# GStreamer/gstreamer

Measured on AMD Instinct MI355X. Metric: 4K frames/s (videoconvertscale NV12->BGRA) per GPU; % HBM roofline, higher is better.
Workload: dtype u8; 1 GPU; C2: 3840x2160 NV12 (bt709 limited, chroma-site mpeg2) -> BGRA, fused unpack + chroma upsample + matrix + pack, 32 frames/step, pools 33 in / 32 out resident in HBM, 1 stream per GPU, 32 frame(s) per kernel launch; plan=fused_convert_pair[NV12->BGRA,h2cs,v2,matrix=ayuv_argb], frames_per_launch=32, parallelism=stream-per-gpu x1

## Files before the change

### gstreamer_amd/csrc/video_scale_col.h

```cpp
#pragma once
#include "video_hscale420.h"

#define GSTAMD_COL_MAX_WAVES 8
#define GSTAMD_COL_MAX_FRAMES 16
#define GSTAMD_COL_FLAG_BYTES 64

namespace gstamd {

struct ColFrames {
  const uint8_t *y[GSTAMD_COL_MAX_FRAMES];
  const uint8_t *c0[GSTAMD_COL_MAX_FRAMES];
  const uint8_t *c1[GSTAMD_COL_MAX_FRAMES];
  uint8_t *dst[GSTAMD_COL_MAX_FRAMES];
};

#ifdef __HIPCC__
typedef __amdgpu_buffer_rsrc_t colplane_t;
#else
struct colplane_t { const uint8_t *p; uint32_t bytes; };
#endif
struct ColSrc {
  colplane_t y, c0, c1;
  colplane_t out;
};
// ... 478 lines not shown
       : "=&v" (w), "=&v" (t01), "=&v" (t23) : "s" (six), "v" (a0), "v" (a1), "v" (a2), "v" (a3));
  return w ^ 0x80808080u;
#else
  const int a[4] = {a0, a1, a2, a3};
  uint32_t w = 0;
  for (int k = 0; k < 4; k++) {
    const int v = ((int) (int16_t) (uint16_t) a[k]) >> 6;
    w |= (uint32_t) (v < 0 ? 0 : (v > 255 ? 255 : v)) << (8 * k);
  }
  return w ^ 0x80808080u;
#endif
}

GSTAMD_HD uint32_t col_fin_px (int ay, int au, int av)
{
#ifdef __HIPCC__
  uint32_t t01 = 0xffu, t23, w;
  const int six = 6;
  asm ("s_nop 2\n\t"
       "v_ashrrev_i16_sdwa %2, %3, %5 dst_sel:WORD_0 dst_unused:UNUSED_PAD src0_sel:DWORD src1_sel:WORD_0\n\t"
       "v_ashrrev_i16_sdwa %1, %3, %4 dst_sel:WORD_1 dst_unused:UNUSED_PRESERVE src0_sel:DWORD src1_sel:WORD_0\n\t"
       "v_ashrrev_i16_sdwa %2, %3, %6 dst_sel:WORD_1 dst_unused:UNUSED_PRESERVE src0_sel:DWORD src1_sel:WORD_0\n\t"
       "v_sat_pk_u8_i16 %0, %1\n\t"
       "v_sat_pk_u8_i16_sdwa %0, %2 dst_sel:WORD_1 dst_unused:UNUSED_PRESERVE src0_sel:DWORD\n\t"
       "s_nop 0"
       : "=&v" (w), "+v" (t01), "=&v" (t23) : "s" (six), "v" (ay), "v" (au), "v" (av));
  return w;
#else
  return 0xffu | (h420r_finish (ay) << 8) | (h420r_finish (au) << 16) | (h420r_finish (av) << 24);
#endif
}

template <int OPL, int NW, int WSTEP, int A8>
GSTAMD_HD void col_hfilter (const ColLane<OPL, NW> &L, const uint8_t *stage, uint32_t gw[3][OPL])
{
  typedef ColGeom<OPL> G;
  constexpr int SH = WSTEP >= 0 ? WSTEP : 0;
  constexpr int NWIN = WSTEP >= 0 ? 1 : OPL;
  constexpr int NWORDS = NW + SH;
  int acc[4][3][OPL];
  uint32_t w[2][3][NWIN][NWORDS];
  auto fetch = [&](int k, uint32_t (*d)[NWIN][NWORDS]) {
#pragma unroll
    for (int c = 0; c < 3; c++)
#pragma unroll
      for (int i = 0; i < NWIN; i++) {
#if defined(GSTAMD_COL_ABL) && GSTAMD_COL_ABL == 2
        for (int q = 0; q < NWORDS; q++)
          d[c][i][q] = (uint32_t) L.lb[k][i] * 3u + q + c;
#else
        col_lds_words<NWORDS, A8> (stage + L.lb[k][i] + c * G::PP, d[c][i]);
#endif
      }
  };
  fetch (0, w[0]);
#pragma unroll
  for (int k = 0; k < 4; k++) {
    if (k < 3)
      fetch (k + 1, w[(k + 1) & 1]);
#pragma unroll
    for (int c = 0; c < 3; c++)
#pragma unroll
      for (int i = 0; i < OPL; i++) {
        const uint32_t *ww = w[k & 1][c][WSTEP >= 0 ? 0 : i] + (WSTEP >= 0 && i ? SH : 0);
        int a = L.hinit[i];
#pragma unroll
        for (int q = 0; q < NW; q++) {
#if defined(GSTAMD_COL_ABL) && GSTAMD_COL_ABL == 5
          a ^= (int) ww[q];
#else
          a = col_dot4 (ww[q], L.tw[i][q], a);
#endif
        }
        acc[k][c][i] = a;
      }
  }
#pragma unroll
  for (int c = 0; c < 3; c++)
#pragma unroll
    for (int i = 0; i < OPL; i++)
      gw[c][i] = col_fin4 (acc[0][c][i], acc[1][c][i], acc[2][c][i], acc[3][c][i]);
}

template <int OPL, int NW, class NB>
GSTAMD_HD void col_hfilter_regs (const ColLane<OPL, NW> &L, NB &nb, uint32_t gw[3][OPL])
{
  static_assert (OPL == 2 && NW <= 4, "register windows: two outputs per lane, windows of up to five words");
  constexpr int NWORDS = NW + 1;
  int acc[4][3][OPL];
#pragma unroll
  for (int k = 0; k < 4; k++)
#pragma unroll
    for (int c = 0; c < 3; c++) {
      uint32_t w[5];
      w[0] = L.win[k][c][0], w[1] = L.win[k][c][1];
      w[2] = nb (w[0], k, c, 0, 1);
      w[3] = NWORDS > 3 ? nb (w[1], k, c, 1, 1) : 0u;
      w[4] = NWORDS > 4 ? nb (w[2], k, c, 0, 2) : 0u;
#pragma unroll
      for (int i = 0; i < OPL; i++) {
        int a = L.hinit[i];
#pragma unroll
        for (int q = 0; q < NW; q++)
          a = col_dot4 (w[q + i], L.tw[i][q], a);
        acc[k][c][i] = a;
      }
    }
#pragma unroll
  for (int c = 0; c < 3; c++)
#pragma unroll
    for (int i = 0; i < OPL; i++)
      gw[c][i] = col_fin4 (acc[0][c][i], acc[1][c][i], acc[2][c][i], acc[3][c][i]);
}

template <int OPL>
GSTAMD_HD void col_slot_store (uint32_t *slot, int lane, const uint32_t gw[3][OPL])
{
#pragma unroll
  for (int c = 0; c < 3; c++) {
    uint32_t *d = slot + (c * 64 + lane) * OPL;
    if constexpr (OPL == 2)
      *(uint2 *) d = gstamd_make_uint2 (gw[c][0], gw[c][1]);
    else
      *d = gw[c][0];
  }
}

template <int OPL>
GSTAMD_HD void col_slot_load (const uint32_t *slot, int lane, uint32_t gw[3][OPL])
{
#pragma unroll
  for (int c = 0; c < 3; c++) {
    const uint32_t *d = slot + (c * 64 + lane) * OPL;
    if constexpr (OPL == 2) {
      const uint2 v = *(const uint2 *) d;
      gw[c][0] = v.x, gw[c][1] = v.y;
    } else {
#ifdef __HIPCC__
      gw[c][0] = *(const __attribute__ ((address_space (3))) uint32_t *) d;
#else
      gw[c][0] = *d;
#endif
    }
  }
}

template <int OPL, int NGV>
GSTAMD_HD void col_ring_put (ColRingRegs<OPL, NGV> &rg, const uint32_t gw[3][OPL])
{
#pragma unroll
  for (int k = 0; k + 1 < NGV; k++)
#pragma unroll
    for (int c = 0; c < 3; c++)
#pragma unroll
      for (int i = 0; i < OPL; i++)
        rg.w[k][c][i] = rg.w[k + 1][c][i];
#pragma unroll
  for (int c = 0; c < 3; c++)
#pragma unroll
    for (int i = 0; i < OPL; i++)
      rg.w[NGV - 1][c][i] = gw[c][i];
}

template <int OPL, int NGV, int POST>
GSTAMD_HD void col_vrow (const ColRingRegs<OPL, NGV> &rg, const uint32_t *e, const ColParams &p, const ColSrc &s, const Dst &dst, const PostFast &pf, int x, int j)
{
  int acc[3][OPL];
#pragma unroll
  for (int c = 0; c < 3; c++)
#pragma unroll
    for (int i = 0; i < OPL; i++)
      acc[c][i] = (int) e[2];
#pragma unroll
  for (int k = 0; k < NGV; k++)
#pragma unroll
    for (int c = 0; c < 3; c++)
#pragma unroll
      for (int i = 0; i < OPL; i++)
        acc[c][i] = col_dot4s (rg.w[k][c][i], e[3 + k], acc[c][i]);
  uint32_t px[OPL];
#pragma unroll
  for (int i = 0; i < OPL; i++) {
    const uint32_t q = col_fin_px (acc[0][i], acc[1][i], acc[2][i]);
    if constexpr (POST) {
      const uint32_t z = q ^ 0x80808080u;
      px[i] = fast_pixel (pf.fp, z, 0x0c01010cu, z, 0x0c02020cu, 0x0c03030cu);
    } else {
      px[i] = dst.final ? pack_px (dst.pack_pos, apply_color (dst.post, q)) : q;
    }
  }
  col_store32 (s.out, (uint32_t) (4 * x), col_row_off (j, p.dstride), px, OPL);
}

struct ColWavePlan {
  int r0, r1;
  int ga, ge, gl, gp;
};

GSTAMD_HD bool col_wave_plan (const ColParams &p, int chunk, int wave, ColWavePlan *w)
{
  const int ra = chunk * p.rows_per_wg, rb = ra + p.rows_per_wg < p.out_h ? ra + p.rows_per_wg : p.out_h;
  w->r0 = ra + wave * p.rows_per_wave;
  if (w->r0 >= rb)
    return false;
  const int mine = wave == p.nwaves - 1 ? p.rows_last : p.rows_per_wave;
  w->r1 = w->r0 + mine < rb ? w->r0 + mine : rb;
  uint32_t e[8];
  col_entry8 (p.vrow, w->r0, e);
  w->ga = (int) e[0];
  col_entry8 (p.vrow, w->r1 - 1, e);
  w->gl = (int) e[1];
  if (w->r1 == rb || p.pubn == 0) {
    w->ge = w->gl + 1;
  } else {
    col_entry8 (p.vrow, w->r1, e);
    w->ge = (int) e[0];
    if (w->ge > w->gl + 1)
      w->ge = w->gl + 1;
  }
  if (w->r0 == ra || p.pubn == 0) {
    w->gp = w->ga - 1;
  } else {
    col_entry8 (p.vrow, w->r0 - 1, e);
    w->gp = (int) e[1];
  }
  return true;
}

template <int OPL, int NW, int NGV, int CH, int SEMI, int WSTEP, int A8, int POST, class X>
GSTAMD_HD void col_wave (X &x, const ColParams &p, const ColSrc &s, const int32_t *tile, const ColWavePlan &wp, uint8_t *wave_lds, uint8_t *below_lds,
    uint32_t *flags, int wave, const Dst &dst, const PostFast &pf)
{
  constexpr int RW = OPL == 2 && WSTEP == 1 && A8 == 2;
  typedef ColGeom<OPL, RW> G;
  typedef ColLane<OPL, NW> Lane;
  typedef ColRaw<OPL> Raw;
  typedef ColRingRegs<OPL, NGV> Ring;
  uint8_t *stage = wave_lds, *craw = wave_lds + G::STAGEB;
  uint32_t *pub = (uint32_t *) (wave_lds + G::STAGEB + GSTAMD_COL_CRAW_BYTES (OPL));
  const uint32_t *pub_below = (const uint32_t *) (below_lds + G::STAGEB + GSTAMD_COL_CRAW_BYTES (OPL));
  const bool aligned = ((tile[3] - tile[2]) % 16) == 0 && tile[3] > 0 && tile[3] + G::SPAN <= p.width;
  x.each ([&](int lane, Lane &L, Raw &ra, Ring &) {
    col_setup<OPL, NW, CH, SEMI, RW> (p, tile, lane, L);
    col_request_chroma<OPL, NW, SEMI> (p, s, L, 2 * wp.ga - 2, ra);
    if (aligned)
      col_stage_loads<OPL, NW, SEMI, 1, RW> (L, ra, stage, craw, false);
    else
      col_stage_loads<OPL, NW, SEMI, 0, RW> (L, ra, stage, craw, false);
    col_request<OPL, NW, SEMI> (p, s, L, wp.ga, ra);
  });
  x.sync ();
  x.each ([&](int, Lane &L, Raw &, Ring &) {
    if (aligned)
      col_first_row<OPL, NW, CH, SEMI, 1> (L, craw);
    else
      col_first_row<OPL, NW, CH, SEMI, 0> (L, craw);
  });
  x.sync ();
  int r = wp.r0;
  uint32_t e[8];
  col_entry8 (p.vrow, r, e);
#ifdef GSTAMD_COL_TRACE
  unsigned long long tacc[8] = {0, 0, 0, 0, 0, 0, 0, 0}, tprev = x.now ();
#define COL_STAMP(k) do { const unsigned long long t_ = x.now (); tacc[k] += t_ - tprev; tprev = t_; } while (0)
#else
#define COL_STAMP(k) do { } while (0)
#endif
  auto rows = [&](int g) {
    while (r < wp.r1 && (int) e[1] == g) {
#if !(defined(GSTAMD_COL_ABL) && GSTAMD_COL_ABL == 3)
      x.each ([&](int, Lane &L, Raw &, Ring &rg) { col_vrow<OPL, NGV, POST> (rg, e, p, s, dst, pf, L.xo, r); });
#endif
      r++;
      if (r < wp.r1)
        col_entry8 (p.vrow, r, e);
    }
  };
  int g = wp.ga;
  COL_STAMP (0);
  while (g < wp.ge) {
    const int gn = g + 1 < wp.ge ? g + 1 : wp.ge - 1;
#ifdef GSTAMD_COL_TRACE
    x.wait_loads ();
    COL_STAMP (1);
#endif
    if (aligned)
      x.each ([&](int, Lane &L, Raw &ra, Ring &) {
        col_stage_loads<OPL, NW, SEMI, 1, RW> (L, ra, stage, craw, true);
        col_request<OPL, NW, SEMI> (p, s, L, gn, ra);
      });
    else
      x.each ([&](int, Lane &L, Raw &ra, Ring &) {
        col_stage_loads<OPL, NW, SEMI, 0, RW> (L, ra, stage, craw, true);
        col_request<OPL, NW, SEMI> (p, s, L, gn, ra);
      });
    x.sync ();
    if (aligned)
      x.each ([&](int, Lane &L, Raw &, Ring &) { col_stage_chroma<OPL, NW, CH, SEMI, 1, RW> (L, craw, stage); });
    else
      x.each ([&](int, Lane &L, Raw &, Ring &) { col_stage_chroma<OPL, NW, CH, SEMI, 0, RW> (L, craw, stage); });
    x.sync ();
    COL_STAMP (2);
    if constexpr (RW) {
      x.each ([&](int, Lane &L, Raw &, Ring &) {
#pragma unroll
        for (int k = 0; k < 4; k++)
          col_lds_words<2, 1> (stage + L.st + k * G::LINEB, L.win[k][0]);
      });
      x.each_nb ([&](int lane, Lane &L, Raw &, Ring &rg, auto &nb) {
        uint32_t gw[3][OPL];
        col_hfilter_regs<OPL, NW> (L, nb, gw);
        col_ring_put<OPL, NGV> (rg, gw);
        if (g <= wp.gp)
          col_slot_store<OPL> (pub + (size_t) (g - wp.ga) * G::SLOTW, lane, gw);
      });
    } else {
      x.each ([&](int lane, Lane &L, Raw &, Ring &rg) {
        uint32_t gw[3][OPL];
        col_hfilter<OPL, NW, WSTEP, A8> (L, stage, gw);
        col_ring_put<OPL, NGV> (rg, gw);
        if (g <= wp.gp)
          col_slot_store<OPL> (pub + (size_t) (g - wp.ga) * G::SLOTW, lane, gw);
      });
    }
    x.sync ();
    if (g == wp.gp)
      x.publish (flags, wave);
    COL_STAMP (3);
    rows (g);
    COL_STAMP (4);
    g++;
  }
  if (wp.gp >= wp.ga)
    x.publish (flags, wave);
  if (wp.gl >= wp.ge) {
    x.wait_flag (flags, wave + 1);
    for (; g <= wp.gl; g++) {
      x.each ([&](int lane, Lane &, Raw &, Ring &rg) {
        uint32_t gw[3][OPL];
        col_slot_load<OPL> (pub_below + (size_t) (g - wp.ge) * G::SLOTW, lane, gw);
        col_ring_put<OPL, NGV> (rg, gw);
      });
      rows (g);
    }
  }
  COL_STAMP (5);
#ifdef GSTAMD_COL_TRACE
  x.trace_out (p.trace, tacc, wp.ge - wp.ga);
#endif
#undef COL_STAMP
}

}
```

### gstreamer_amd/csrc/video_fast.h

```cpp
#pragma once
#include "video_device.h"

namespace gstamd {

struct FastParams {
  int width, height;
  int p8[5];
  uint32_t pack_sel;
  int u_first;
  int pc[5];
  int crow_lo, crow_hi;
  int pack_pos[4];
  int px_bytes;
  const uint8_t *lut;
  int lut_keep;
  MatrixParams m8;
  int ayuv;
  int store_policy;
};

#ifdef __HIPCC__
extern __shared__ uint32_t fast_lut_lds[];
#else
static uint32_t fast_lut_lds[64];
// ... 205 lines not shown
#ifdef __HIPCC__
  uint32_t r;
  asm ("v_sat_pk_u8_i16 %0, %1" : "=v" (r) : "v" (v));
  return r;
#else
  const int a = (int16_t) (v & 0xffff), b = (int16_t) (v >> 16);
  return (uint32_t) (a < 0 ? 0 : a > 255 ? 255 : a) | ((uint32_t) (b < 0 ? 0 : b > 255 ? 255 : b) << 8);
#endif
}

GSTAMD_HD int add_hiwords (int pa, int pb)
{
#ifdef __HIPCC__
  int r;
  asm ("v_add_u32_sdwa %0, sext(%1), sext(%2) dst_sel:DWORD dst_unused:UNUSED_PAD src0_sel:WORD_1 src1_sel:WORD_1" : "=v" (r) : "v" (pa), "v" (pb));
  return r;
#else
  return (pa >> 16) + (pb >> 16);
#endif
}

template <int W>
GSTAMD_HD void add_hiwords_into (uint32_t &dst, int pa, int pb)
{
#ifdef __HIPCC__
  if (W == 0)
    asm ("v_add_u32_sdwa %0, sext(%1), sext(%2) dst_sel:WORD_0 dst_unused:UNUSED_PRESERVE src0_sel:WORD_1 src1_sel:WORD_1" : "+v" (dst) : "v" (pa), "v" (pb));
  else
    asm ("v_add_u32_sdwa %0, sext(%1), sext(%2) dst_sel:WORD_1 dst_unused:UNUSED_PRESERVE src0_sel:WORD_1 src1_sel:WORD_1" : "+v" (dst) : "v" (pa), "v" (pb));
#else
  const uint32_t r = (uint32_t) ((pa >> 16) + (pb >> 16)) & 0xffffu;
  dst = W == 0 ? (dst & 0xffff0000u) | r : (dst & 0x0000ffffu) | (r << 16);
#endif
}

GSTAMD_HD void sat_pk_u8_hi (uint32_t &dst, uint32_t v)
{
#ifdef __HIPCC__
  asm ("v_sat_pk_u8_i16_sdwa %0, %1 dst_sel:WORD_1 dst_unused:UNUSED_PRESERVE src0_sel:DWORD" : "+v" (dst) : "v" (v));
#else
  dst = (dst & 0xffffu) | (sat_pk_u8 (v) << 16);
#endif
}

GSTAMD_HD uint32_t pk_mad (uint32_t a, uint32_t k_splat, uint32_t c)
{
#ifdef __HIPCC__
  uint32_t r;
  asm ("v_pk_mad_u16 %0, %1, %2, %3" : "=v" (r) : "v" (a), "s" (k_splat), "v" (c));
  return r;
#else
  const uint32_t lo = ((a & 0xffffu) * (k_splat & 0xffffu) + (c & 0xffffu)) & 0xffffu;
  const uint32_t hi = ((a >> 16) * (k_splat >> 16) + (c >> 16)) & 0xffffu;
  return lo | (hi << 16);
#endif
}

GSTAMD_HD void blend_rows_hi (uint32_t a, uint32_t b, uint32_t &x0, uint32_t &x1)
{
  x0 = pk_mad (a, 0x00c000c0u, pk_mad (b, 0x00400040u, 0x80808080u));
  x1 = pk_mad (b, 0x00c000c0u, pk_mad (a, 0x00400040u, 0x80808080u));
}

#define GSTAMD_LAYOUT(pr, pg, pb) ((pr) | ((pg) << 2) | ((pb) << 4))
#define GSTAMD_LAYOUT_AYUV GSTAMD_LAYOUT (0, 0, 4)
#define GSTAMD_AYUV_X80(ys, c) ((bperm ((c), (ys), 0x0604000cu) ^ 0x80808000u) | 0xffu)
#define GSTAMD_AYUV_OUT(fp, px) ((fp).ayuv == 2 ? apply_matrix ((fp).m8, (px)) : (px))

template <int L>
GSTAMD_HD void layout_init (uint32_t (&q)[4][2])
{
  constexpr int PA = (L & GSTAMD_LAYOUT_AYUV) ? 0 : 6 - (L & 3) - ((L >> 2) & 3) - ((L >> 4) & 3);
#pragma unroll
  for (int j = 0; j < 4; j++) {
    q[j][0] = q[j][1] = 0;
    q[j][PA >> 1] = 255u << (16 * (PA & 1));
#ifdef __HIPCC__
    asm volatile ("" : "+v" (q[j][0]), "+v" (q[j][1]));
#endif
  }
}

template <int L, int ABL>
GSTAMD_HD void fast_emit4_l (const FastParams &fp, uint8_t *__restrict__ d, bool store, uint32_t yw, const uint32_t *xh, uint32_t (&q)[4][2])
{
  constexpr int PR = L & 3, PG = (L >> 2) & 3, PB = (L >> 4) & 3;
  uint32_t o[4];
  if (ABL == 1) {
#pragma unroll
    for (int j = 0; j < 4; j++)
      o[j] = yw ^ xh[j];
  } else {
    const uint32_t yx = yw ^ 0x80808080u;
    const uint32_t ys01 = bperm (yx, yx, 0x01010000u), ys23 = bperm (yx, yx, 0x03030202u);
    const uint32_t csel = fp.u_first ? 0x03030101u : 0x01010303u;
    uint32_t cs[4];
    int wy[4], prv[4], pbu[4], pgu[4], pgv[4], g0[4];
#pragma unroll
    for (int j = 0; j < 4; j++)
      cs[j] = bperm (xh[j], xh[j], csel);
    wy[0] = mul_word<0> (ys01, fp.pc[0]) + 0x00800000;
    wy[1] = mul_word<1> (ys01, fp.pc[0]) + 0x00800000;
    wy[2] = mul_word<0> (ys23, fp.pc[0]) + 0x00800000;
    wy[3] = mul_word<1> (ys23, fp.pc[0]) + 0x00800000;
#pragma unroll
    for (int j = 0; j < 4; j++)
      pgu[j] = mul_word<0> (cs[j], fp.pc[3]);
#pragma unroll
    for (int j = 0; j < 4; j++)
      prv[j] = mul_word<1> (cs[j], fp.pc[1]);
#pragma unroll
    for (int j = 0; j < 4; j++)
      g0[j] = add_hiwords (wy[j], pgu[j]);
#pragma unroll
    for (int j = 0; j < 4; j++)
      pgv[j] = mul_word<1> (cs[j], fp.pc[4]);
#pragma unroll
    for (int j = 0; j < 4; j++)
      add_hiwords_into<PR & 1> (q[j][PR >> 1], wy[j], prv[j]);
#pragma unroll
    for (int j = 0; j < 4; j++)
      pbu[j] = mul_word<0> (cs[j], fp.pc[2]);
#pragma unroll
    for (int j = 0; j < 4; j++)
      add_hiword_into<PG & 1> (q[j][PG >> 1], g0[j], pgv[j]);
#pragma unroll
    for (int j = 0; j < 4; j++)
      add_hiwords_into<PB & 1> (q[j][PB >> 1], wy[j], pbu[j]);
#pragma unroll
    for (int j = 0; j < 4; j++)
      o[j] = sat_pk_u8 (q[j][0]);
#pragma unroll
    for (int j = 0; j < 4; j++)
      sat_pk_u8_hi (o[j], q[j][1]);
  }
  if (ABL == GSTAMD_FAST_LUT) {
#pragma unroll
    for (int j = 0; j < 4; j++)
      o[j] = fast_lut3_px (o[j], fp.lut_keep);
  }
  if (store) {
    if (fp.px_bytes == 3)
      store12_stream (d, o[0], o[1], o[2], o[3]);
    else
      store16_policy (d, o[0], o[1], o[2], o[3], fp.store_policy);
  }
}

template <int CH>
GSTAMD_HD void chroma_filter4 (uint32_t raw, uint32_t nxt, uint32_t prv_hi, uint32_t *out)
{
  const uint32_t s1 = bperm (raw, raw, 0x0c010c00u), s2 = bperm (raw, raw, 0x0c030c02u);
  if (CH == CHROMA_H_NONE) {
    out[0] = out[1] = s1;
    out[2] = out[3] = s2;
    return;
  }
  const uint32_t s3 = bperm (nxt, nxt, 0x0c010c00u);
  if (CH == CHROMA_H_H2_CS) {
    out[0] = s1;
    out[1] = pk_shr<1> (s1 + s2 + 0x00010001u);
    out[2] = s2;
    out[3] = pk_shr<1> (s2 + s3 + 0x00010001u);
  } else {
    const uint32_t s0 = bperm (prv_hi, prv_hi, 0x0c030c02u);
    out[0] = pk_shr<2> (s0 + 3u * s1 + 0x00020002u);
    out[1] = pk_shr<2> (3u * s1 + s2 + 0x00020002u);
    out[2] = pk_shr<2> (s1 + 3u * s2 + 0x00020002u);
    out[3] = pk_shr<2> (3u * s2 + s3 + 0x00020002u);
  }
}

struct ChromaRaw4 {
  uint32_t raw, nxt, prv_hi;
};

struct __attribute__ ((aligned (4))) u32x2u { uint32_t a, b; };

GSTAMD_HD uint32_t load_stream32 (const uint8_t *__restrict__ p)
{
#ifdef __HIPCC__
  return __builtin_nontemporal_load ((const uint32_t *) p);
#else
  return *(const uint32_t *) p;
#endif
}

template <int CH>
GSTAMD_HD void chroma_load4 (const uint8_t *__restrict__ row, int cw, int x0, ChromaRaw4 &r)
{
  const int k0 = x0 >> 1;
  const uint8_t *p = row + 2 * (size_t) k0;
  r.nxt = r.prv_hi = 0;
  if (CH != CHROMA_H_NONE && k0 + 2 < cw) {
    const u32x2u m = *(const u32x2u *) p;
    r.raw = m.a;
    r.nxt = m.b;
  } else {
    r.raw = *(const uint32_t *) p;
    if (CH != CHROMA_H_NONE)
      r.nxt = *(const uint16_t *) (row + 2 * (size_t) (cw - 1));
  }
  if (CH == CHROMA_H_H2)
    r.prv_hi = (uint32_t) * (const uint16_t *) (row + 2 * (size_t) (k0 > 0 ? k0 - 1 : 0)) << 16;
}

template <int CH, int L, int ABL>
GSTAMD_HD void fast_strip (const FastParams &fp, const Planes &pl, uint8_t *__restrict__ dst, int dstride, int x0, int p_begin,
    int p_end)
{
  const int w = fp.width, h = fp.height, cw = (w + 1) >> 1;
  const uint8_t *yb = pl.p[0] + x0, *cbase = pl.p[1];
  const int ys = pl.stride[0], cs = pl.stride[1];
  uint8_t *db = dst + (size_t) fp.px_bytes * (size_t) x0;
  uint32_t q[4][2];
  layout_init<L> (q);

  uint32_t cprev[4], ccur[4], c0[4], c1[4];
  ChromaRaw4 craw;
  uint32_t y0, y1;
  {
    ChromaRaw4 r0;
    chroma_load4<CH> (cbase + (ptrdiff_t) (p_begin - 1 > fp.crow_lo ? p_begin - 1 : fp.crow_lo) * cs, cw, x0, r0);
    chroma_filter4<CH> (r0.raw, r0.nxt, r0.prv_hi, cprev);
  }
  {
    const int p = p_begin, l0 = 2 * p - 1, l1 = 2 * p;
    chroma_load4<CH> (cbase + (ptrdiff_t) (p < fp.crow_hi ? p : fp.crow_hi) * cs, cw, x0, craw);
    y0 = load_stream32 (yb + (size_t) (l0 >= 0 ? l0 : 0) * ys);
    y1 = load_stream32 (yb + (size_t) (l1 < h ? l1 : h - 1) * ys);
  }
  for (int p = p_begin; p < p_end; p++) {
    const int l0 = 2 * p - 1, l1 = 2 * p;
    const bool have0 = l0 >= 0, have1 = l1 < h;
    const uint32_t cy0 = y0, cy1 = y1;
    const ChromaRaw4 cr_now = craw;
    if (p + 1 < p_end) {
      const int pn = p + 1, n0 = 2 * pn - 1, n1 = 2 * pn;
      chroma_load4<CH> (cbase + (ptrdiff_t) (pn < fp.crow_hi ? pn : fp.crow_hi) * cs, cw, x0, craw);
      y0 = load_stream32 (yb + (size_t) n0 * ys);
      y1 = load_stream32 (yb + (size_t) (n1 < h ? n1 : h - 1) * ys);
    }
    chroma_filter4<CH> (cr_now.raw, cr_now.nxt, cr_now.prv_hi, ccur);
#pragma unroll
    for (int j = 0; j < 4; j++)
      blend_rows_hi (cprev[j], ccur[j], c0[j], c1[j]);
    fast_emit4_l<L, ABL> (fp, db + (size_t) (have0 ? l0 : l1) * dstride, have0, cy0, c0, q);
    fast_emit4_l<L, ABL> (fp, db + (size_t) (have1 ? l1 : l0) * dstride, have1, cy1, c1, q);
#pragma unroll
    for (int i = 0; i < 4; i++)
      cprev[i] = ccur[i];
  }
}

#define GSTAMD_WIDE_PX 1024
struct WideLds {
  uint32_t y[2][256];
  uint32_t c[2][4 + 256 + 4];
};

#ifdef __HIPCC__
typedef unsigned int gstamd_u32x4 __attribute__ ((ext_vector_type (4)));
#endif

template <bool STREAM>
GSTAMD_HD void wide_load16 (const uint8_t *__restrict__ p, int nd, bool vec, uint32_t *out)
{
  if (nd >= 4 && vec) {
#ifdef __HIPCC__
    const gstamd_u32x4 v = STREAM ? __builtin_nontemporal_load ((const gstamd_u32x4 *) p) : *(const gstamd_u32x4 *) p;
    out[0] = v.x;
    out[1] = v.y;
    out[2] = v.z;
    out[3] = v.w;
#else
    const uint4 v = *(const uint4 *) p;
    out[0] = v.x;
    out[1] = v.y;
    out[2] = v.z;
    out[3] = v.w;
#endif
  } else {
#pragma unroll
    for (int j = 0; j < 4; j++)
      out[j] = j < nd ? *(const uint32_t *) (p + 4 * j) : 0u;
  }
}

GSTAMD_HD void wide_put16 (uint32_t *l, const uint32_t *v)
{
  *(uint4 *) l = gstamd_make_uint4 (v[0], v[1], v[2], v[3]);
}

struct WideRegs {
  uint32_t y0[4], y1[4], c[4];
  uint32_t cn, cp;
};

template <int CH>
GSTAMD_HD void wide_fetch_chroma (const FastParams &fp, const Planes &pl, int xw, int crow, int lane, bool vec, WideRegs &r)
{
  const int w = fp.width, xl = xw + 16 * lane;
  if (xl >= w)
    return;
  const int nd = (w - xl) >> 2;
  const uint8_t *row = pl.p[1] + (ptrdiff_t) crow * pl.stride[1];
  wide_load16<false> (row + xl, nd, vec, r.c);
  if (CH != CHROMA_H_NONE && (lane == 63 || nd <= 4)) {
    const int xn = xl + 4 * (nd < 4 ? nd : 4);
    r.cn = xn < w ? *(const uint32_t *) (row + xn) : (uint32_t) * (const uint16_t *) (row + w - 2);
  }
  if (CH == CHROMA_H_H2 && lane == 0)
    r.cp = xw > 0 ? *(const uint32_t *) (row + xw - 4) : 0u;
}

template <int CH>
GSTAMD_HD void wide_commit_chroma (const FastParams &fp, int xw, int lane, const WideRegs &r, uint32_t *crow_lds)
{
  const int w = fp.width, xl = xw + 16 * lane;
  if (xl >= w)
    return;
  const int nd = (w - xl) >> 2;
  wide_put16 (&crow_lds[4 + 4 * lane], r.c);
  if (CH != CHROMA_H_NONE && (lane == 63 || nd <= 4))
    crow_lds[4 + 4 * lane + (nd < 4 ? nd : 4)] = r.cn;
  if (CH == CHROMA_H_H2 && lane == 0)
    crow_lds[3] = xw > 0 ? r.cp : r.c[0] << 16;
}

template <int CH>
GSTAMD_HD void wide_fetch (const FastParams &fp, const Planes &pl, int xw, int p, int lane, bool vec, WideRegs &r)
{
  const int w = fp.width, h = fp.height;
  const int xl = xw + 16 * lane;
  if (xl >= w)
    return;
  const int nd = (w - xl) >> 2;
// ... 60 lines not shown
```

### gstreamer_amd/csrc/video_kernels.hip

```cpp
#include <hip/hip_runtime.h>
#include <algorithm>
#include <cstdio>
#include <cstdlib>
#include <stdint.h>
#include <stdio.h>
#include <stdlib.h>
#include <string.h>

#include "planner.h"
#include "tuning.h"
#include "video_kernels.h"
#include "video_device.h"
#include "video_fast.h"
#include "video_scale_fast.h"
#include "video_hscale420.h"
#include "video_pack.h"
#include "video_bilinear_fast.h"
#include "video_encode_fast.h"
#include "video_planes.h"
#include "video_deep.h"
#include "video_dither.h"
#include "video_dither_ed.h"
#include "video_relayout.h"
#include "video_swizzle34.h"
// ... 1259 lines not shown
  if (vec_ok) {
    vec_ok = aligned (pl.p[0], 8) && (pl.stride[0] % 8) == 0;
    if (f.kind == UNPACK_SEMI)
      vec_ok = vec_ok && aligned (pl.p[1], 8) && (pl.stride[1] % 8) == 0;
    else
      vec_ok = vec_ok && aligned (pl.p[1], 4) && aligned (pl.p[2], 4) && (pl.stride[1] % 4) == 0 && (pl.stride[2] % 4) == 0;
  }
  if (f.kind == UNPACK_PACKED4 && aligned (dst, 16) && (dstride % 16) == 0 && aligned (pl.p[0], 16) && (pl.stride[0] % 16) == 0)
    vec_ok = 2;
  const int bx = spans >= 256 ? 256 : (spans > 64 ? 128 : 64);
  dim3 grid ((spans + bx - 1) / bx, f.height + extra_rows), block (bx);
  switch (f.chroma_h) {
    case CHROMA_H_H2_CS:
      hipLaunchKernelGGL (k_convert<CHROMA_H_H2_CS>, grid, block, 0, stream, f, pl, vpair_dev, color, pack_pos[0],
          pack_pos[1], pack_pos[2], pack_pos[3], dst, dstride, spans, vec_ok);
      break;
    case CHROMA_H_H2:
      hipLaunchKernelGGL (k_convert<CHROMA_H_H2>, grid, block, 0, stream, f, pl, vpair_dev, color, pack_pos[0],
          pack_pos[1], pack_pos[2], pack_pos[3], dst, dstride, spans, vec_ok);
      break;
    default:
      hipLaunchKernelGGL (k_convert<CHROMA_H_NONE>, grid, block, 0, stream, f, pl, vpair_dev, color, pack_pos[0],
          pack_pos[1], pack_pos[2], pack_pos[3], dst, dstride, spans, vec_ok);
      break;
  }
  return hipGetLastError ();
}

template <int CH>
static hipError_t launch_convert_gamma_ch (const FrontParams &f, const Planes &pl, const int *vpair_dev, const ColorParams &color, const int pack_pos[4],
    uint8_t *dst, int dstride, int spans, int vec_ok, const GammaDev &g, hipStream_t stream)
{
  const void *fn = (const void *) k_convert_gamma<CH>;
  hipError_t e = hipFuncSetAttribute (fn, hipFuncAttributeMaxDynamicSharedMemorySize, GSTAMD_GAMMA_LDS_BYTES);
  if (e != hipSuccess)
    return e;
  static int n_cu = 0;
  if (n_cu == 0) {
    int dev = 0;
    hipDeviceProp_t prop;
    n_cu = hipGetDevice (&dev) == hipSuccess && hipGetDeviceProperties (&prop, dev) == hipSuccess && prop.multiProcessorCount > 0 ? prop.multiProcessorCount : 256;
  }
  const int gx = (spans + 511) / 512;
  int rows = g.comp ? 2 : (f.height * gx + 2 * n_cu - 1) / (2 * n_cu);
  rows = rows < 1 ? 1 : rows;
  dim3 grid (gx, (f.height + rows - 1) / rows);
  hipLaunchKernelGGL (k_convert_gamma<CH>, grid, dim3 (512), g.comp ? 256 : GSTAMD_GAMMA_LDS_BYTES, stream, f, pl, vpair_dev, color, pack_pos[0], pack_pos[1], pack_pos[2],
      pack_pos[3], dst, dstride, spans, vec_ok, g, rows);
  return hipGetLastError ();
}

hipError_t launch_convert_gamma (const FrontParams &f, const Planes &pl, const int *vpair_dev, const ColorParams &color, const int pack_pos[4], uint8_t *dst,
    int dstride, const GammaDev &g, hipStream_t stream)
{
  video_frame_list_touch (dst);
  const int spans = (f.width + K1_PX - 1) / K1_PX;
  int vec_ok = aligned (dst, 16) && (dstride % 16) == 0 && kind_has_planes (f.kind) && f.w_sub == 1;
  if (vec_ok) {
    vec_ok = aligned (pl.p[0], 8) && (pl.stride[0] % 8) == 0;
    if (f.kind == UNPACK_SEMI)
      vec_ok = vec_ok && aligned (pl.p[1], 8) && (pl.stride[1] % 8) == 0;
    else
      vec_ok = vec_ok && aligned (pl.p[1], 4) && aligned (pl.p[2], 4) && (pl.stride[1] % 4) == 0 && (pl.stride[2] % 4) == 0;
  }
  if (f.kind == UNPACK_PACKED4 && aligned (dst, 16) && (dstride % 16) == 0 && aligned (pl.p[0], 16) && (pl.stride[0] % 16) == 0)
    vec_ok = 2;
  if (f.chroma_h == CHROMA_H_H2_CS)
    return launch_convert_gamma_ch<CHROMA_H_H2_CS> (f, pl, vpair_dev, color, pack_pos, dst, dstride, spans, vec_ok, g, stream);
  if (f.chroma_h == CHROMA_H_H2)
    return launch_convert_gamma_ch<CHROMA_H_H2> (f, pl, vpair_dev, color, pack_pos, dst, dstride, spans, vec_ok, g, stream);
  return launch_convert_gamma_ch<CHROMA_H_NONE> (f, pl, vpair_dev, color, pack_pos, dst, dstride, spans, vec_ok, g, stream);
}

template <int CH, int L, int ABL>
__global__ __launch_bounds__ (64) void k_convert_strip (FastParams fp, FrameBatch batch, int pairs, int K)
{
  if (ABL == GSTAMD_FAST_LUT) {
    fast_lut_lds[threadIdx.x] = ((const uint32_t *) fp.lut)[threadIdx.x];
    __syncthreads ();
  }
  const Planes pl = batch_planes (batch, blockIdx.z);
  const int x0 = (blockIdx.x * 64 + threadIdx.x) * 4;
  const int p0 = blockIdx.y * K;
  if (x0 + 4 <= fp.width)
    fast_strip<CH, L, ABL> (fp, pl, batch.dst[blockIdx.z], batch.dstride, x0, p0, p0 + K < pairs ? p0 + K : pairs);
}

template <int CH, int L, int ABL>
__global__ __launch_bounds__ (64) void k_convert_strip_xcd (FastParams fp, FrameBatch batch, int ncol, int pairs, int K, int strips, int total_strips)
{
  if (ABL == GSTAMD_FAST_LUT) {
    fast_lut_lds[threadIdx.x] = ((const uint32_t *) fp.lut)[threadIdx.x];
    __syncthreads ();
  }
  int col, S;
  if (!wide_block_map (blockIdx.x, ncol, total_strips, &col, &S))
    return;
  const int z = S / strips, p0 = (S - z * strips) * K;
  const Planes pl = batch_planes (batch, z);
  const int x0 = (col * 64 + threadIdx.x) * 4;
  if (x0 + 4 <= fp.width)
    fast_strip<CH, L, ABL> (fp, pl, batch.dst[z], batch.dstride, x0, p0, p0 + K < pairs ? p0 + K : pairs);
}

static int fast_layout (const FastParams &fp)
{
  return fp.ayuv ? GSTAMD_LAYOUT_AYUV : GSTAMD_LAYOUT (fp.pack_pos[1], fp.pack_pos[2], fp.pack_pos[3]);
}

#define GSTAMD_FOR_LAYOUTS(W) \
    W (2, 1, 0)       \
    W (0, 1, 2)       \
    W (1, 2, 3)       \
    W (3, 2, 1)

template <int CH, int ABL>
static bool launch_strip_variant (const FastParams &fp, const FrameBatch &batch, int n, int K, bool xcd_order, hipStream_t stream)
{
  const int pairs = fp.height / 2 + 1, strips = (pairs + K - 1) / K, ncol = (fp.width + 255) / 256;
#define W(pr, pg, pb) case GSTAMD_LAYOUT (pr, pg, pb): \
    if (xcd_order) \
      hipLaunchKernelGGL ((k_convert_strip_xcd<CH, GSTAMD_LAYOUT (pr, pg, pb), ABL>), dim3 (wide_grid_blocks (ncol, strips * n)), dim3 (64), ABL == GSTAMD_FAST_LUT ? 256 : 0, stream, \
          fp, batch, ncol, pairs, K, strips, strips * n); \
    else \
      hipLaunchKernelGGL ((k_convert_strip<CH, GSTAMD_LAYOUT (pr, pg, pb), ABL>), dim3 (ncol, strips, n), dim3 (64), ABL == GSTAMD_FAST_LUT ? 256 : 0, stream, fp, batch, pairs, K); \
    return true;
  switch (fast_layout (fp)) {
    GSTAMD_FOR_LAYOUTS (W)
  }
#undef W
  return false;
}

template <int CH, int L, int ABL>
__global__ __launch_bounds__ (64) void k_convert_wide (FastParams fp, FrameBatch batch, int nxb, int pairs, int K, int strips, int total_strips,
    int vec)
{
  __shared__ WideLds lds;
  int xb, S;
  if (!wide_block_map (blockIdx.x, nxb, total_strips, &xb, &S))
    return;
  const int z = S / strips, p0 = (S - z * strips) * K, p1 = p0 + K < pairs ? p0 + K : pairs;
  const Planes pl = batch_planes (batch, z);
  const int xw = xb * GSTAMD_WIDE_PX, lane = threadIdx.x;
  const bool v = vec != 0;
  WideRegs r;
  wide_fetch_chroma<CH> (fp, pl, xw, p0 - 1 > fp.crow_lo ? p0 - 1 : fp.crow_lo, lane, v, r);
  wide_commit_chroma<CH> (fp, xw, lane, r, lds.c[0]);
  wide_fetch<CH> (fp, pl, xw, p0, lane, v, r);
  for (int p = p0; p < p1; p++) {
    const int k = p - p0;
    wide_commit<CH> (fp, xw, lane, r, &lds, (k + 1) & 1);
    __syncthreads ();
    if (p + 1 < p1)
      wide_fetch<CH> (fp, pl, xw, p + 1, lane, v, r);
    wide_emit<CH, L, ABL> (fp, batch.dst[z], batch.dstride, xw, p, lane, &lds, k & 1);
    __syncthreads ();
  }
}

static bool wide_vec_ok (const FrameBatch &batch, int n)
{
  bool ok = (batch.ystride % 16) == 0 && (batch.uvstride % 16) == 0;
  for (int i = 0; i < n; i++)
    ok = ok && aligned (batch.y[i], 16) && aligned (batch.uv[i], 16);
  return ok;
}

template <int CH, int ABL>
static bool launch_wide_variant (const FastParams &fp, const FrameBatch &batch, int n, int K, hipStream_t stream)
{
  const int pairs = fp.height / 2 + 1, nxb = (fp.width + GSTAMD_WIDE_PX - 1) / GSTAMD_WIDE_PX;
  const int strips = (pairs + K - 1) / K;
  const int blocks = wide_grid_blocks (nxb, strips * n);
  const int vec = wide_vec_ok (batch, n) ? 1 : 0;
#define W(pr, pg, pb) case GSTAMD_LAYOUT (pr, pg, pb): \
    hipLaunchKernelGGL ((k_convert_wide<CH, GSTAMD_LAYOUT (pr, pg, pb), ABL>), dim3 (blocks), dim3 (64), 0, stream, fp, batch, nxb, pairs, K, strips, strips * n, vec); \
    return true;
  switch (fast_layout (fp)) {
    GSTAMD_FOR_LAYOUTS (W)
  }
#undef W
  return false;
}

struct FastVariant { int set, shape, abl, K, order; };
static const FastVariant &fast_variant ()
{
  static FastVariant v = {-1, 0, 0, 0, 0};
  if (v.set < 0) {
    const char *e = tuning_text ("GSTAMD_FAST_VARIANT");
    v.set = e && sscanf (e, "%d,%d,%d,%d", &v.shape, &v.abl, &v.K, &v.order) >= 1;
  }
  return v;
}

template <int CH>
static bool launch_fast (const FastParams &fp, const FrameBatch &batch, int n, hipStream_t stream)
{
  const FastVariant &v = fast_variant ();
  const int k_default = n == 1 && (long) fp.width * fp.height < 6000000L ? 2 : 3;
  const int shape = v.set ? v.shape : 0, K = v.set && v.K > 0 ? v.K : k_default;
#ifdef GSTAMD_TUNING
  if (v.set && v.abl && CH == CHROMA_H_H2_CS)
    return shape == 1 ? launch_wide_variant<CHROMA_H_H2_CS, 1> (fp, batch, n, K, stream) :
        launch_strip_variant<CHROMA_H_H2_CS, 1> (fp, batch, n, K, v.order != 0, stream);
#endif
  if (fp.lut)
    return launch_strip_variant<CH, GSTAMD_FAST_LUT> (fp, batch, n, K, v.set && v.order != 0, stream);
  if (shape == 1 && fp.width >= GSTAMD_WIDE_PX / 2 && fp.px_bytes == 4)
    return launch_wide_variant<CH, 0> (fp, batch, n, K, stream);
  return launch_strip_variant<CH, 0> (fp, batch, n, K, v.set && v.order != 0, stream);
}

hipError_t launch_convert_pair (const FastParams &fp_in, int chroma_h, const uint8_t *y, const uint8_t *uv, uint8_t *dst, int ystride, int uvstride,
    int dstride, hipStream_t stream)
{
  int n_frames;
  const FrameDeltas &fl = video_frame_list_peek (y, dst, &n_frames);
  const int dalign = fp_in.px_bytes == 3 ? 4 : 16;
  for (int i = 1; i < n_frames; i++)
    if (fl.s[i] % 4 != 0 || fl.d[i] % dalign != 0)
      n_frames = 1;
  if (n_frames > 1)
    (void) frame_list_for (y, dst, &n_frames);
  else
    video_frame_list_touch (dst);
  FastParams fpl = fp_in;
  {
    const int pin = tuning_int ("GSTAMD_STORE_POLICY", -1);
    const int few = tuning_int ("GSTAMD_STORE_WT_BELOW", 9);
    fpl.store_policy = pin >= 0 ? pin : (n_frames < few ? 1 : 3);
  }
  const FastParams &fp = fpl;
  for (int base = 0; base < n_frames; base += GSTAMD_MAX_BATCH) {
    const int n = n_frames - base < GSTAMD_MAX_BATCH ? n_frames - base : GSTAMD_MAX_BATCH;
    FrameBatch batch;
    memset (&batch, 0, sizeof (batch));
    for (int i = 0; i < n; i++) {
      batch.y[i] = y + fl.s[base + i];
      batch.uv[i] = uv + fl.s[base + i];
      batch.dst[i] = dst + fl.d[base + i];
    }
    batch.ystride = ystride;
    batch.uvstride = uvstride;
    batch.dstride = dstride;
    bool ok;
    switch (chroma_h) {
      case CHROMA_H_H2_CS:
        ok = launch_fast<CHROMA_H_H2_CS> (fp, batch, n, stream);
        break;
      case CHROMA_H_H2:
        ok = launch_fast<CHROMA_H_H2> (fp, batch, n, stream);
        break;
      default:
        ok = launch_fast<CHROMA_H_NONE> (fp, batch, n, stream);
        break;
    }
    if (!ok)
      return hipErrorInvalidValue;
  }
  return hipGetLastError ();
}

static int front_vec_ok (const FrontParams &f, const Planes &pl)
{
  if (!kind_has_planes (f.kind) || f.w_sub != 1)
    return 0;
  int ok = aligned (pl.p[0], 8) && (pl.stride[0] % 8) == 0;
  if (f.kind == UNPACK_SEMI)
    ok = ok && aligned (pl.p[1], 8) && (pl.stride[1] % 8) == 0;
  else
    ok = ok && aligned (pl.p[1], 4) && aligned (pl.p[2], 4) && (pl.stride[1] % 4) == 0 && (pl.stride[2] % 4) == 0;
  return ok;
}

static int front_packed_ok (const SrcFront &s)
{
  return s.vec_ok && s.f.w_sub == 1 && kind_has_planes (s.f.kind) && s.pre.matrix.kind == MATRIX_NONE && s.pre.alpha_kind == ALPHA_NONE;
}

static int dot4_source_ok (const SrcFront &s)
{
  return (kind_has_planes (s.f.kind) || (s.f.kind == UNPACK_PACKED422 && s.f.hi_depth == 0)) && s.pre.matrix.kind == MATRIX_NONE && s.pre.alpha_kind == ALPHA_NONE;
// ... 581 lines not shown
```

Before: 135,500 frames/s.

## Hand-schedule horizontal dot4 with DPP shifts and rotate ring by phase

Replaces the compiler-generated horizontal filter in the register-window path with inline assembly. It processes two rows per call using v_dot4c with DPP wave_shl:1, so the neighbor words come from DPP instead of separate cross-lane moves. It also removes the register shift in the vertical ring by unrolling the group loop over ring phases, so each group writes its slot in place and the vertical filter indexes it modulo NGV. Code size grows from the phase unrolling. The hand-written asm hardcodes the DPP shift semantics and an s_nop hazard wait, and may not match the old nb neighbor function in every configuration.

```diff
diff --git a/gstreamer_amd/csrc/video_scale_col.h b/gstreamer_amd/csrc/video_scale_col.h
--- a/gstreamer_amd/csrc/video_scale_col.h
+++ b/gstreamer_amd/csrc/video_scale_col.h
@@ -584,30 +584,76 @@
       gw[c][i] = col_fin4 (acc[0][c][i], acc[1][c][i], acc[2][c][i], acc[3][c][i]);
 }
 
+#ifdef __HIPCC__
+#define GSTAMD_COL_SHL1 " wave_shl:1 row_mask:0xf bank_mask:0xf bound_ctrl:1\n\t"
+#define GSTAMD_COL_HPAIR_HEAD \
+  "v_dot4_i32_i8 %[a0], %[wa0], %[t00], %[h0]\n\t" \
+  "v_dot4_i32_i8 %[b0], %[wb0], %[t00], %[h0]\n\t" \
+  "v_dot4_i32_i8 %[a1], %[wa1], %[t10], %[h1]\n\t" \
+  "v_dot4_i32_i8 %[b1], %[wb1], %[t10], %[h1]\n\t" \
+  "v_dot4c_i32_i8_e32 %[a0], %[wa1], %[t01]\n\t" \
+  "v_dot4c_i32_i8_e32 %[b0], %[wb1], %[t01]\n\t" \
+  "v_mov_b32_dpp %[wa2], %[wa0]" GSTAMD_COL_SHL1 \
+  "v_mov_b32_dpp %[wb2], %[wb0]" GSTAMD_COL_SHL1 \
+  "v_dot4c_i32_i8_e32 %[a1], %[wa2], %[t11]\n\t" \
+  "v_dot4c_i32_i8_e32 %[b1], %[wb2], %[t11]\n\t" \
+  "v_dot4c_i32_i8_e32 %[a0], %[wa2], %[t02]\n\t" \
+  "v_dot4c_i32_i8_e32 %[b0], %[wb2], %[t02]\n\t" \
+  "v_dot4c_i32_i8_dpp %[a1], %[wa1], %[t12]" GSTAMD_COL_SHL1 \
+  "v_dot4c_i32_i8_dpp %[b1], %[wb1], %[t12]" GSTAMD_COL_SHL1
+#define GSTAMD_COL_HPAIR_TAIL4 \
+  "v_dot4c_i32_i8_dpp %[a0], %[wa1], %[t03]" GSTAMD_COL_SHL1 \
+  "v_dot4c_i32_i8_dpp %[b0], %[wb1], %[t03]" GSTAMD_COL_SHL1 \
+  "v_dot4c_i32_i8_dpp %[a1], %[wa2], %[t13]" GSTAMD_COL_SHL1 \
+  "v_dot4c_i32_i8_dpp %[b1], %[wb2], %[t13]" GSTAMD_COL_SHL1
+#define GSTAMD_COL_HPAIR_OUT [a0] "=&v" (a0), [b0] "=&v" (b0), [a1] "=&v" (a1), [b1] "=&v" (b1), [wa2] "=&v" (wa2), [wb2] "=&v" (wb2)
+#define GSTAMD_COL_HPAIR_IN \
+  [wa0] "v" (L.win[ka][c][0]), [wa1] "v" (L.win[ka][c][1]), [wb0] "v" (L.win[kb][c][0]), [wb1] "v" (L.win[kb][c][1]), [h0] "v" (L.hinit[0]), \
+  [h1] "v" (L.hinit[1]), [t00] "v" (L.tw[0][0]), [t01] "v" (L.tw[0][1]), [t02] "v" (L.tw[0][2]), [t10] "v" (L.tw[1][0]), [t11] "v" (L.tw[1][1]), [t12] "v" (L.tw[1][2])
+#endif
+template <int NW, class NB>
+GSTAMD_HD void col_hpair (const ColLane<2, NW> &L, NB &nb, int ka, int kb, int c, int acc[4][3][2])
+{
+  static_assert (NW == 3 || NW == 4, "register windows: windows of four or five words");
+#ifdef __HIPCC__
+  (void) nb;
+  int a0, a1, b0, b1;
+  uint32_t wa2, wb2;
+  if constexpr (NW == 4)
+    asm (GSTAMD_COL_HPAIR_HEAD GSTAMD_COL_HPAIR_TAIL4 "s_nop 2"
+         : GSTAMD_COL_HPAIR_OUT : GSTAMD_COL_HPAIR_IN, [t03] "v" (L.tw[0][NW - 1]), [t13] "v" (L.tw[1][NW - 1]));
+  else
+    asm (GSTAMD_COL_HPAIR_HEAD "s_nop 2" : GSTAMD_COL_HPAIR_OUT : GSTAMD_COL_HPAIR_IN);
+  acc[ka][c][0] = a0, acc[ka][c][1] = a1, acc[kb][c][0] = b0, acc[kb][c][1] = b1;
+#else
+  for (int k = ka;; k = kb) {
+    uint32_t w[5];
+    w[0] = L.win[k][c][0], w[1] = L.win[k][c][1];
+    w[2] = nb (w[0], k, c, 0, 1);
+    w[3] = nb (w[1], k, c, 1, 1);
+    w[4] = NW > 3 ? nb (w[2], k, c, 0, 2) : 0u;
+    for (int i = 0; i < 2; i++) {
+      int a = L.hinit[i];
+      for (int q = 0; q < NW; q++)
+        a = dot4_i8 (w[q + i], L.tw[i][q], a);
+      acc[k][c][i] = a;
+    }
+    if (k == kb)
+      break;
+  }
+#endif
+}
+
 template <int OPL, int NW, class NB>
 GSTAMD_HD void col_hfilter_regs (const ColLane<OPL, NW> &L, NB &nb, uint32_t gw[3][OPL])
 {
-  static_assert (OPL == 2 && NW <= 4, "register windows: two outputs per lane, windows of up to five words");
-  constexpr int NWORDS = NW + 1;
+  static_assert (OPL == 2, "register windows: two outputs per lane");
   int acc[4][3][OPL];
 #pragma unroll
-  for (int k = 0; k < 4; k++)
-#pragma unroll
-    for (int c = 0; c < 3; c++) {
-      uint32_t w[5];
-      w[0] = L.win[k][c][0], w[1] = L.win[k][c][1];
-      w[2] = nb (w[0], k, c, 0, 1);
-      w[3] = NWORDS > 3 ? nb (w[1], k, c, 1, 1) : 0u;
-      w[4] = NWORDS > 4 ? nb (w[2], k, c, 0, 2) : 0u;
-#pragma unroll
-      for (int i = 0; i < OPL; i++) {
-        int a = L.hinit[i];
-#pragma unroll
-        for (int q = 0; q < NW; q++)
-          a = col_dot4 (w[q + i], L.tw[i][q], a);
-        acc[k][c][i] = a;
-      }
-    }
+  for (int c = 0; c < 3; c++) {
+    col_hpair<NW> (L, nb, 0, 1, c, acc);
+    col_hpair<NW> (L, nb, 2, 3, c, acc);
+  }
 #pragma unroll
   for (int c = 0; c < 3; c++)
 #pragma unroll
@@ -647,24 +693,32 @@
   }
 }
 
-template <int OPL, int NGV>
+template <int PH>
+struct ColPhase { static constexpr int value = PH; };
+
+template <int FROM, int N, class F>
+GSTAMD_HD bool col_phases (F &f)
+{
+  if constexpr (FROM < N) {
+    if (!f (ColPhase<FROM> ()))
+      return false;
+    return col_phases<FROM + 1, N> (f);
+  } else {
+    return true;
+  }
+}
+
+template <int OPL, int NGV, int PH>
 GSTAMD_HD void col_ring_put (ColRingRegs<OPL, NGV> &rg, const uint32_t gw[3][OPL])
 {
 #pragma unroll
-  for (int k = 0; k + 1 < NGV; k++)
-#pragma unroll
-    for (int c = 0; c < 3; c++)
-#pragma unroll
-      for (int i = 0; i < OPL; i++)
-        rg.w[k][c][i] = rg.w[k + 1][c][i];
-#pragma unroll
   for (int c = 0; c < 3; c++)
 #pragma unroll
     for (int i = 0; i < OPL; i++)
-      rg.w[NGV - 1][c][i] = gw[c][i];
-}
-
-template <int OPL, int NGV, int POST>
+      rg.w[PH][c][i] = gw[c][i];
+}
+
+template <int OPL, int NGV, int POST, int PH>
 GSTAMD_HD void col_vrow (const ColRingRegs<OPL, NGV> &rg, const uint32_t *e, const ColParams &p, const ColSrc &s, const Dst &dst, const PostFast &pf, int x, int j)
 {
   int acc[3][OPL];
@@ -679,7 +733,7 @@
     for (int c = 0; c < 3; c++)
 #pragma unroll
       for (int i = 0; i < OPL; i++)
-        acc[c][i] = col_dot4s (rg.w[k][c][i], e[3 + k], acc[c][i]);
+        acc[c][i] = col_dot4s (rg.w[(PH + 1 + k) % NGV][c][i], e[3 + k], acc[c][i]);
   uint32_t px[OPL];
 #pragma unroll
   for (int i = 0; i < OPL; i++) {
@@ -768,19 +822,26 @@
 #else
 #define COL_STAMP(k) do { } while (0)
 #endif
-  auto rows = [&](int g) {
+  auto rows = [&](auto ph, int g) {
+    typedef decltype (ph) PH;
     while (r < wp.r1 && (int) e[1] == g) {
 #if !(defined(GSTAMD_COL_ABL) && GSTAMD_COL_ABL == 3)
-      x.each ([&](int, Lane &L, Raw &, Ring &rg) { col_vrow<OPL, NGV, POST> (rg, e, p, s, dst, pf, L.xo, r); });
+      x.each ([&](int, Lane &L, Raw &, Ring &rg) { col_vrow<OPL, NGV, POST, PH::value> (rg, e, p, s, dst, pf, L.xo, r); });
 #endif
       r++;
       if (r < wp.r1)
         col_entry8 (p.vrow, r, e);
     }
   };
-  int g = wp.ga;
+  static_assert (NGV >= 3 && NGV <= 4, "the hand-over's switch below has a case per ring phase");
+  int g = wp.ga, phase = 0;
   COL_STAMP (0);
-  while (g < wp.ge) {
+  auto make = [&](auto ph) -> bool {
+    typedef decltype (ph) PH;
+    if (g >= wp.ge) {
+      phase = PH::value;
+      return false;
+    }
     const int gn = g + 1 < wp.ge ? g + 1 : wp.ge - 1;
 #ifdef GSTAMD_COL_TRACE
     x.wait_loads ();
@@ -812,7 +873,7 @@
       x.each_nb ([&](int lane, Lane &L, Raw &, Ring &rg, auto &nb) {
         uint32_t gw[3][OPL];
         col_hfilter_regs<OPL, NW> (L, nb, gw);
-        col_ring_put<OPL, NGV> (rg, gw);
+        col_ring_put<OPL, NGV, PH::value> (rg, gw);
         if (g <= wp.gp)
           col_slot_store<OPL> (pub + (size_t) (g - wp.ga) * G::SLOTW, lane, gw);
       });
@@ -820,7 +881,7 @@
       x.each ([&](int lane, Lane &L, Raw &, Ring &rg) {
         uint32_t gw[3][OPL];
         col_hfilter<OPL, NW, WSTEP, A8> (L, stage, gw);
-        col_ring_put<OPL, NGV> (rg, gw);
+        col_ring_put<OPL, NGV, PH::value> (rg, gw);
         if (g <= wp.gp)
           col_slot_store<OPL> (pub + (size_t) (g - wp.ga) * G::SLOTW, lane, gw);
       });
@@ -829,21 +890,38 @@
     if (g == wp.gp)
       x.publish (flags, wave);
     COL_STAMP (3);
-    rows (g);
+    rows (ph, g);
     COL_STAMP (4);
     g++;
+    return true;
+  };
+  while (col_phases<0, NGV> (make)) {
   }
   if (wp.gp >= wp.ga)
     x.publish (flags, wave);
   if (wp.gl >= wp.ge) {
     x.wait_flag (flags, wave + 1);
-    for (; g <= wp.gl; g++) {
+    auto take = [&](auto ph) -> bool {
+      typedef decltype (ph) PH;
+      if (g > wp.gl)
+        return false;
       x.each ([&](int lane, Lane &, Raw &, Ring &rg) {
         uint32_t gw[3][OPL];
         col_slot_load<OPL> (pub_below + (size_t) (g - wp.ge) * G::SLOTW, lane, gw);
-        col_ring_put<OPL, NGV> (rg, gw);
+        col_ring_put<OPL, NGV, PH::value> (rg, gw);
       });
-      rows (g);
+      rows (ph, g);
+      g++;
+      return true;
+    };
+    bool more = true;
+    switch (phase) {
+      case 1: more = col_phases<1, NGV> (take); break;
+      case 2: more = col_phases<2, NGV> (take); break;
+      case 3: more = col_phases<3, NGV> (take); break;
+      default: break;
+    }
+    while (more && col_phases<0, NGV> (take)) {
     }
   }
   COL_STAMP (5);
```

After: 133,000 frames/s. 0.982x the previous value.

## Add interior fast path with buffer stores and unguarded loads for strip kernel

Applied to the files above, without the earlier changes.

Adds a specialized interior-strip path for 4-byte output without LUT. It drops the row clamping and boundary checks, uses AMDGPU raw buffer 128-bit stores with write-through cache policy bits, and places scheduling barriers to control instruction interleaving. It also lowers the default rows-per-strip K to 2 for straight 4-byte conversions, which raises block count but adds more halo chroma reloads. Edge strips fall back to the existing generic path.

```diff
diff --git a/gstreamer_amd/csrc/video_fast.h b/gstreamer_amd/csrc/video_fast.h
--- a/gstreamer_amd/csrc/video_fast.h
+++ b/gstreamer_amd/csrc/video_fast.h
@@ -311,10 +311,9 @@
 }
 
 template <int L, int ABL>
-GSTAMD_HD void fast_emit4_l (const FastParams &fp, uint8_t *__restrict__ d, bool store, uint32_t yw, const uint32_t *xh, uint32_t (&q)[4][2])
+GSTAMD_HD void fast_px4_l (const FastParams &fp, uint32_t yw, const uint32_t *xh, uint32_t (&q)[4][2], uint32_t (&o)[4])
 {
   constexpr int PR = L & 3, PG = (L >> 2) & 3, PB = (L >> 4) & 3;
-  uint32_t o[4];
   if (ABL == 1) {
 #pragma unroll
     for (int j = 0; j < 4; j++)
@@ -368,6 +367,13 @@
     for (int j = 0; j < 4; j++)
       o[j] = fast_lut3_px (o[j], fp.lut_keep);
   }
+}
+
+template <int L, int ABL>
+GSTAMD_HD void fast_emit4_l (const FastParams &fp, uint8_t *__restrict__ d, bool store, uint32_t yw, const uint32_t *xh, uint32_t (&q)[4][2])
+{
+  uint32_t o[4];
+  fast_px4_l<L, ABL> (fp, yw, xh, q, o);
   if (store) {
     if (fp.px_bytes == 3)
       store12_stream (d, o[0], o[1], o[2], o[3]);
@@ -482,6 +488,109 @@
   }
 }
 
+GSTAMD_HD bool fast_strip_is_interior (const FastParams &fp, int dstride, int col, int p_begin, int p_end)
+{
+  const int cw = (fp.width + 1) >> 1;
+  return fp.px_bytes == 4 && p_begin >= 1 && p_end > p_begin && 2 * (p_end - 1) < fp.height
+      && p_begin - 1 >= fp.crow_lo && p_end - 1 <= fp.crow_hi
+      && col * 128 + 128 < cw
+      && dstride > 0 && (long long) fp.height * dstride < 0x7fffffffLL;
+}
+
+#ifdef __HIPCC__
+template <int POLICY>
+__device__ __forceinline__ void store16_buffer (__amdgpu_buffer_rsrc_t rsrc, uint32_t lane_off, uint32_t line_off, const uint32_t (&o)[4])
+{
+  typedef unsigned int u32x4 __attribute__ ((ext_vector_type (4)));
+  static_assert (POLICY == 1 || POLICY == 3, "the write-through policies only");
+  const u32x4 v = {o[0], o[1], o[2], o[3]};
+  __builtin_amdgcn_raw_buffer_store_b128 (v, rsrc, lane_off + line_off, 0, POLICY == 1 ? (1 | 16) : (1 | 2 | 16));
+}
+
+template <int CH>
+__device__ __forceinline__ void chroma_load4_inner (const uint8_t *__restrict__ row, int x0, ChromaRaw4 &r)
+{
+  const int k0 = x0 >> 1;
+  const uint8_t *p = row + 2 * (size_t) k0;
+  r.nxt = r.prv_hi = 0;
+  if (CH != CHROMA_H_NONE) {
+    const u32x2u m = *(const u32x2u *) p;
+    r.raw = m.a;
+    r.nxt = m.b;
+  } else
+    r.raw = *(const uint32_t *) p;
+  if (CH == CHROMA_H_H2)
+    r.prv_hi = (uint32_t) * (const uint16_t *) (row + 2 * (size_t) (k0 > 0 ? k0 - 1 : 0)) << 16;
+}
+
+template <int CH, int L, int ABL, int POLICY>
+__device__ __forceinline__ void fast_strip_interior (const FastParams &fp, const Planes &pl, uint8_t *__restrict__ dst, int dstride, int x0, int p_begin,
+    int p_end)
+{
+  const uint8_t *yb = pl.p[0] + x0, *cbase = pl.p[1];
+  const int ys = pl.stride[0], cs = pl.stride[1];
+  const __amdgpu_buffer_rsrc_t rsrc = __builtin_amdgcn_make_buffer_rsrc (dst, 0, (fp.height - 1) * dstride + 4 * fp.width, 0x00020000);
+  const uint32_t lane_off = 4u * (uint32_t) x0;
+  uint32_t q[4][2];
+  layout_init<L> (q);
+
+  uint32_t cprev[4], ccur[4], c0[4], c1[4], o0[4], o1[4];
+  ChromaRaw4 craw, r0;
+  uint32_t y0, y1;
+  chroma_load4_inner<CH> (cbase + (ptrdiff_t) (p_begin - 1) * cs, x0, r0);
+  chroma_load4_inner<CH> (cbase + (ptrdiff_t) p_begin * cs, x0, craw);
+  y0 = load_stream32 (yb + (size_t) (2 * p_begin - 1) * ys);
+  y1 = load_stream32 (yb + (size_t) (2 * p_begin) * ys);
+  chroma_filter4<CH> (r0.raw, r0.nxt, r0.prv_hi, cprev);
+  asm volatile ("" : "+v" (y0), "+v" (y1), "+v" (craw.raw), "+v" (craw.nxt), "+v" (craw.prv_hi));
+  uint32_t line_off = (uint32_t) (2 * p_begin - 1) * (uint32_t) dstride;
+  for (int p = p_begin; p + 1 < p_end; p++) {
+    const uint32_t cy0 = y0, cy1 = y1;
+    const ChromaRaw4 cr_now = craw;
+    chroma_load4_inner<CH> (cbase + (ptrdiff_t) (p + 1) * cs, x0, craw);
+    y0 = load_stream32 (yb + (size_t) (2 * p + 1) * ys);
+    y1 = load_stream32 (yb + (size_t) (2 * p + 2) * ys);
+    chroma_filter4<CH> (cr_now.raw, cr_now.nxt, cr_now.prv_hi, ccur);
+#pragma unroll
+    for (int j = 0; j < 4; j++)
+      blend_rows_hi (cprev[j], ccur[j], c0[j], c1[j]);
+    fast_px4_l<L, ABL> (fp, cy0, c0, q, o0);
+    store16_buffer<POLICY> (rsrc, lane_off, line_off, o0);
+    __builtin_amdgcn_sched_barrier (0);
+    fast_px4_l<L, ABL> (fp, cy1, c1, q, o1);
+    store16_buffer<POLICY> (rsrc, lane_off, line_off + (uint32_t) dstride, o1);
+    line_off += 2u * (uint32_t) dstride;
+#pragma unroll
+    for (int i = 0; i < 4; i++)
+      cprev[i] = ccur[i];
+    __builtin_amdgcn_sched_barrier (0);
+    asm volatile ("" : "+v" (y0), "+v" (y1), "+v" (craw.raw), "+v" (craw.nxt), "+v" (craw.prv_hi));
+  }
+  chroma_filter4<CH> (craw.raw, craw.nxt, craw.prv_hi, ccur);
+#pragma unroll
+  for (int j = 0; j < 4; j++)
+    blend_rows_hi (cprev[j], ccur[j], c0[j], c1[j]);
+  fast_px4_l<L, ABL> (fp, y0, c0, q, o0);
+  store16_buffer<POLICY> (rsrc, lane_off, line_off, o0);
+  fast_px4_l<L, ABL> (fp, y1, c1, q, o1);
+  store16_buffer<POLICY> (rsrc, lane_off, line_off + (uint32_t) dstride, o1);
+}
+
+template <int CH, int L, int ABL>
+__device__ __forceinline__ void fast_strip_wave (const FastParams &fp, const Planes &pl, uint8_t *__restrict__ dst, int dstride, int col, int x0, int p_begin,
+    int p_end)
+{
+  if (ABL == 0 && fast_strip_is_interior (fp, dstride, col, p_begin, p_end)) {
+    if (fp.store_policy == 1)
+      return fast_strip_interior<CH, L, ABL, 1> (fp, pl, dst, dstride, x0, p_begin, p_end);
+    if (fp.store_policy == 3)
+      return fast_strip_interior<CH, L, ABL, 3> (fp, pl, dst, dstride, x0, p_begin, p_end);
+  }
+  if (x0 + 4 <= fp.width)
+    fast_strip<CH, L, ABL> (fp, pl, dst, dstride, x0, p_begin, p_end);
+}
+#endif
+
 #define GSTAMD_WIDE_PX 1024
 struct WideLds {
   uint32_t y[2][256];
diff --git a/gstreamer_amd/csrc/video_kernels.hip b/gstreamer_amd/csrc/video_kernels.hip
--- a/gstreamer_amd/csrc/video_kernels.hip
+++ b/gstreamer_amd/csrc/video_kernels.hip
@@ -1365,8 +1365,7 @@
   const Planes pl = batch_planes (batch, blockIdx.z);
   const int x0 = (blockIdx.x * 64 + threadIdx.x) * 4;
   const int p0 = blockIdx.y * K;
-  if (x0 + 4 <= fp.width)
-    fast_strip<CH, L, ABL> (fp, pl, batch.dst[blockIdx.z], batch.dstride, x0, p0, p0 + K < pairs ? p0 + K : pairs);
+  fast_strip_wave<CH, L, ABL> (fp, pl, batch.dst[blockIdx.z], batch.dstride, blockIdx.x, x0, p0, p0 + K < pairs ? p0 + K : pairs);
 }
 
 template <int CH, int L, int ABL>
@@ -1382,8 +1381,7 @@
   const int z = S / strips, p0 = (S - z * strips) * K;
   const Planes pl = batch_planes (batch, z);
   const int x0 = (col * 64 + threadIdx.x) * 4;
-  if (x0 + 4 <= fp.width)
-    fast_strip<CH, L, ABL> (fp, pl, batch.dst[z], batch.dstride, x0, p0, p0 + K < pairs ? p0 + K : pairs);
+  fast_strip_wave<CH, L, ABL> (fp, pl, batch.dst[z], batch.dstride, col, x0, p0, p0 + K < pairs ? p0 + K : pairs);
 }
 
 static int fast_layout (const FastParams &fp)
@@ -1482,7 +1480,8 @@
 static bool launch_fast (const FastParams &fp, const FrameBatch &batch, int n, hipStream_t stream)
 {
   const FastVariant &v = fast_variant ();
-  const int k_default = n == 1 && (long) fp.width * fp.height < 6000000L ? 2 : 3;
+  const bool straight = fp.px_bytes == 4 && !fp.lut;
+  const int k_default = straight || (n == 1 && (long) fp.width * fp.height < 6000000L) ? 2 : 3;
   const int shape = v.set ? v.shape : 0, K = v.set && v.K > 0 ? v.K : k_default;
 #ifdef GSTAMD_TUNING
   if (v.set && v.abl && CH == CHROMA_H_H2_CS)
```

After: 133,000 frames/s before, 137,200 frames/s after (median of 6 runs). +3.1%, better.
